# ansonb/RECON

Hardware: AMD Instinct MI355X
Metric: edges aggregated/sec (GAT fwd+bwd) on synthetic KG-context graphs (higher is better)
Workload: dtype f32

## Files before the change

include/recon_hip.h:

```cpp
#ifndef RECON_HIP_H
#define RECON_HIP_H

#include <stddef.h>
#include <stdint.h>

#ifdef __cplusplus
extern "C" {
#endif

#define RECON_ABI_VERSION 2

enum {
    RECON_OK = 0,
    RECON_ERR_INVALID = -1,
    RECON_ERR_UNSUPPORTED = -2,
    RECON_ERR_LAUNCH = -3,
    RECON_ERR_WORKSPACE = -4
};

typedef void* recon_stream_t;

int recon_version(void);
const char* recon_error_string(int code);

// ... 108 lines not shown
typedef struct {
    int32_t N, E;
    int32_t F, R, D, H;
    int32_t concat;
    float alpha;
    const float* x;
    const float* edge_embed;
    const float* a;
    const float* a_2;
    const float* keep;
    float* u;
    float* c_node;
    float* c_rel;
    float* V;
    float* sigma;
    float* Z;
    float* Zk;
    float* out;
    int32_t ld_out;
    void* a_split;
    int32_t split_mode;
    float keep_max;
    void* aux;
    const int32_t* ee_index;
    int32_t ee_rows;
    int32_t io_bf16;
} recon_gat_atp_args;
int recon_gat_atp_bf16_io_supported(int32_t F, int32_t R, int32_t D, int32_t H);

size_t recon_gat_atp_split_bytes(int32_t F, int32_t R, int32_t D, int32_t H);
int recon_gat_atp_f16x2_supported(int32_t F, int32_t R, int32_t D, int32_t H);
int recon_gat_atp_supported(int32_t N, int32_t E, int32_t F, int32_t R, int32_t D, int32_t H);
int32_t recon_gat_atp_instance(int32_t F, int32_t R, int32_t H);
int recon_gat_atp_fwd(const recon_graph* g, const recon_gat_atp_args* args, recon_stream_t stream);
int recon_gat_atp_scores(const recon_graph* g, const recon_gat_atp_args* args, recon_stream_t stream);
int recon_gat_atp_aggregate(const recon_graph* g, const recon_gat_atp_args* args, recon_stream_t stream);
int recon_gat_atp_project(const recon_graph* g, const recon_gat_atp_args* args, recon_stream_t stream);

typedef struct {
    recon_gat_atp_args fwd;
    const float* grad_out;
    int32_t ld_gout;
    float* g_h;
    float* g_V;
    float* g_sigma;
    float* Gxs;
    float* gxd;
    float* Gs;
    float* g_u;
    float* q;
    float* partial;
    float* partial2;
    float* g_x;
    float* g_edge_embed;
    float* g_a;
    float* g_a_2;
    void* gh_split;
    int32_t g_ee_bf16;
} recon_gat_atp_bwd_args;
int recon_gat_atp_bwd_gee_bf16_supported(int32_t F, int32_t R, int32_t D, int32_t H);

size_t recon_gat_atp_bwd_split_bytes(int32_t N, int32_t D, int32_t H);

size_t recon_gat_atp_bwd_partial_floats(int32_t N, int32_t E, int32_t F, int32_t R, int32_t D, int32_t H);
size_t recon_gat_atp_bwd_partial2_floats(int32_t N, int32_t E, int32_t F, int32_t R, int32_t D, int32_t H);
int recon_gat_atp_bwd_ride_plan(int32_t NR, int32_t N, int32_t E, int32_t F, int32_t R, int32_t D, int32_t H, int32_t* plan );
// ... 449 lines not shown
```

recon_amd/_lib.py:

```python
import ctypes as C
import os

_HERE = os.path.dirname(os.path.abspath(__file__))
LIB_PATH = os.environ.get("RECON_HIP_LIB") or os.path.join(_HERE, "csrc", "librecon_hip.so")

ERRORS = {0: "ok", -1: "invalid argument", -2: "unsupported shape", -3: "kernel launch failed",
          -4: "workspace too small"}

c_f32p = C.c_void_p
c_i32p = C.c_void_p
c_i64p = C.c_void_p


class ReconGraph(C.Structure):
    _fields_ = [("N", C.c_int32), ("E", C.c_int32),
                ("rowptr_dst", c_i32p), ("eid", c_i32p), ("src", c_i32p), ("dst", c_i32p),
                ("rowptr_src", c_i32p), ("slot_by_src", c_i32p),
                ("hub_chunk", C.c_int32), ("n_hub", C.c_int32), ("n_piece", C.c_int32),
                ("hub_node", c_i32p), ("hub_ptr", c_i32p), ("piece", c_i32p),
                ("n_hub_src", C.c_int32), ("n_piece_src", C.c_int32), ("hub_node_src", c_i32p), ("hub_ptr_src", c_i32p), ("piece_src", c_i32p),
                ("hub_ws", c_f32p), ("hub_ws_floats", C.c_int64),
                ("n_rows", C.c_int32), ("row_node", c_i32p), ("rowptr_rows", c_i32p), ("node_row", c_i32p)]


# ... 108 lines not shown
    ("recon_error_string", C.c_char_p, [C.c_int]),
    ("recon_graph_workspace_bytes", C.c_size_t, [C.c_int32, C.c_int32]),
    ("recon_graph_build", C.c_int, [c_i64p, c_i64p, C.POINTER(ReconGraph), C.c_void_p, C.c_size_t, C.c_void_p]),
    ("recon_graph_hubs_count", C.c_int, [C.POINTER(ReconGraph), C.c_int32, C.c_void_p, C.POINTER(C.c_int32), C.c_void_p]),
    ("recon_graph_build_checked", C.c_int, [c_i64p, c_i64p, C.POINTER(ReconGraph), C.c_void_p, C.c_size_t, C.c_void_p, C.c_void_p]),
    ("recon_graph_hubs_count_checked", C.c_int, [C.POINTER(ReconGraph), C.c_int32, C.c_void_p, C.POINTER(C.c_int32), C.c_void_p, C.POINTER(C.c_int32), C.c_void_p]),
    ("recon_graph_build_counted", C.c_int, [c_i64p, c_i64p, C.POINTER(ReconGraph), C.c_void_p, C.c_size_t, C.c_void_p, C.c_int32, C.c_void_p]),
    ("recon_graph_hubs_read", C.c_int, [C.POINTER(ReconGraph), C.c_void_p, C.POINTER(C.c_int32), C.c_void_p, C.POINTER(C.c_int32), C.c_void_p]),
    ("recon_graph_hubs_fill", C.c_int, [C.POINTER(ReconGraph), C.c_void_p]),
    ("recon_graph_counts_read", C.c_int, [C.POINTER(ReconGraph), C.c_void_p, C.POINTER(C.c_int32), C.POINTER(C.c_int32), C.c_void_p, C.POINTER(C.c_int32), C.c_void_p]),
    ("recon_graph_rows_compact", C.c_int, [C.POINTER(ReconGraph), C.c_void_p]),
    ("recon_edges_prune_batch", C.c_int, [C.c_void_p, C.c_int32, C.c_void_p, C.c_void_p, C.c_int64, C.c_void_p, C.c_int64, C.c_int32, C.c_void_p, C.c_void_p,
                                          C.c_void_p, C.c_void_p, C.c_void_p, C.c_void_p, C.c_void_p, C.c_void_p, C.c_int64, C.c_void_p]),
    ("recon_gat_atp_bwd_gee_bf16_supported", C.c_int, [C.c_int32, C.c_int32, C.c_int32, C.c_int32]),
    ("recon_slot_index", C.c_int, [C.c_void_p, C.c_void_p, C.c_int32, C.c_void_p, C.c_void_p, C.c_void_p]),
    ("recon_edges_prune", C.c_int, [C.c_void_p, C.c_void_p, C.c_int64, C.c_void_p, C.c_void_p, C.c_int64, C.c_void_p, C.c_int32, C.c_void_p, C.c_void_p,
                                    C.c_void_p, C.c_void_p, C.c_void_p, C.c_void_p, C.c_void_p, C.c_void_p]),
    ("recon_rows_expand", C.c_int, [C.c_void_p, C.c_int32, C.c_void_p, C.c_int32, C.c_int32, C.c_void_p, C.c_int32, C.c_void_p]),
    ("recon_graph_hub_ws_floats", C.c_size_t, [C.POINTER(ReconGraph), C.c_int32, C.c_int32, C.c_int32]),
    ("recon_spmm_rowsum_workspace_floats", C.c_size_t, [C.c_int32, C.c_int32]),
    ("recon_spmm_rowsum_fwd", C.c_int, [C.POINTER(ReconGraph), c_f32p, C.c_int32, c_f32p, c_f32p, C.c_void_p]),
    ("recon_spmm_rowsum_mod_fwd", C.c_int, [C.POINTER(ReconGraph), c_f32p, C.c_int32, C.c_int32, c_f32p, c_f32p, C.c_void_p]),
    ("recon_gather_rows_pair_fwd", C.c_int, [c_f32p, c_i64p, C.c_int64, C.c_int32, c_f32p, C.c_void_p]),
    ("recon_spmm_rowsum_bwd", C.c_int, [c_i64p, C.c_int64, c_f32p, C.c_int32, c_f32p, C.c_void_p]),
    ("recon_gat_fwd", C.c_int, [C.POINTER(ReconGraph), C.POINTER(GatFwdArgs), C.c_void_p]),
    ("recon_gat_project", C.c_int, [C.POINTER(ReconGraph), C.POINTER(GatFwdArgs), C.c_void_p]),
    ("recon_gat_edge_fwd", C.c_int, [C.POINTER(ReconGraph), C.POINTER(GatFwdArgs), C.c_void_p]),
    ("recon_gat_edge_instance", C.c_int32, [C.c_int32] * 2),
    ("recon_gat_bwd_partial_floats", C.c_size_t, [C.c_int32] * 6),
    ("recon_gat_bwd", C.c_int, [C.POINTER(ReconGraph), C.POINTER(GatBwdArgs), C.c_void_p]),
    ("recon_gat_atp_supported", C.c_int, [C.c_int32] * 6),
    ("recon_gat_atp_f16x2_supported", C.c_int, [C.c_int32] * 4),
    ("recon_gat_atp_instance", C.c_int32, [C.c_int32] * 3),
    ("recon_gat_atp_fwd", C.c_int, [C.POINTER(ReconGraph), C.POINTER(GatAtpArgs), C.c_void_p]),
    ("recon_gat_atp_scores", C.c_int, [C.POINTER(ReconGraph), C.POINTER(GatAtpArgs), C.c_void_p]),
    ("recon_gat_atp_aggregate", C.c_int, [C.POINTER(ReconGraph), C.POINTER(GatAtpArgs), C.c_void_p]),
    ("recon_gat_atp_project", C.c_int, [C.POINTER(ReconGraph), C.POINTER(GatAtpArgs), C.c_void_p]),
    ("recon_gat_atp_bwd_partial_floats", C.c_size_t, [C.c_int32] * 6),
    ("recon_gat_atp_bwd_partial2_floats", C.c_size_t, [C.c_int32] * 6),
    ("recon_gat_atp_bwd_ride_plan", C.c_int, [C.c_int32] * 7 + [C.POINTER(C.c_int32)]),
    ("recon_gat_atp_bwd", C.c_int, [C.POINTER(ReconGraph), C.POINTER(GatAtpBwdArgs), C.c_void_p]),
    ("recon_gat_atp_bwd_phase", C.c_int, [C.POINTER(ReconGraph), C.POINTER(GatAtpBwdArgs), C.c_int32, C.c_void_p]),
    ("recon_block_adjacency_fwd", C.c_int, [c_f32p, c_f32p, C.c_int32, C.c_int32, C.c_int32, c_f32p, C.c_void_p]),
    ("recon_block_adjacency_bwd_workspace_floats", C.c_size_t, [C.c_int32] * 3),
    ("recon_block_adjacency_bwd", C.c_int, [c_f32p, C.c_int32, C.c_int32, C.c_int32, c_f32p, c_f32p, c_f32p, C.c_void_p]),
    ("recon_propagate_fwd", C.c_int, [C.POINTER(PropArgs), C.c_void_p]),
    ("recon_propagate_bwd", C.c_int, [C.POINTER(PropBwdArgs), C.c_void_p]),
    ("recon_propagate_form", C.c_int, [C.POINTER(PropArgs)]),
    ("recon_propagate_instance", C.c_int32, [C.POINTER(PropArgs)]),
    ("recon_propagate_bwd_instance", C.c_int32, [C.POINTER(PropBwdArgs)]),
    ("recon_propagate_b16_instance", C.c_int32, [C.POINTER(PropB16Args), C.c_int32]),
    ("recon_propagate_identity_ws_floats", C.c_size_t, [C.c_int32]),
    ("recon_propagate_ws_bytes", C.c_size_t, [C.POINTER(PropArgs)]),
    ("recon_propagate_bwd_ws_floats", C.c_size_t, [C.POINTER(PropArgs)]),
    ("recon_propagate_bwd_chain_ws_floats", C.c_size_t, [C.POINTER(PropArgs)]),
    ("recon_propagate_b16_form", C.c_int, [C.POINTER(PropB16Args)]),
    ("recon_propagate_b16_fwd", C.c_int, [C.POINTER(PropB16Args), C.c_void_p]),
    ("recon_propagate_b16_bwd", C.c_int, [C.POINTER(PropB16BwdArgs), C.c_void_p]),
    ("recon_propagate_b16_bwd_diag_elems", C.c_size_t, [C.POINTER(PropB16Args)]),
    ("recon_block_adjacency_b16_fwd", C.c_int, [C.c_void_p, C.c_void_p, C.c_int32, C.c_int32, C.c_int32, C.c_void_p, C.c_void_p]),
    ("recon_block_adjacency_b16_bwd_workspace_floats", C.c_size_t, [C.c_int32]),
    ("recon_block_adjacency_b16_bwd", C.c_int, [C.c_void_p, C.c_int32, C.c_int32, C.c_int32, C.c_void_p, C.c_void_p, c_f32p, C.c_void_p]),
    ("recon_rel_rows_mm", C.c_int, [C.c_void_p] * 4 + [C.c_int32] * 4 + [C.c_void_p] * 2),
    ("recon_rel_rows_mm_wgrad", C.c_int, [C.c_void_p] * 4 + [C.c_int32] * 3 + [C.c_void_p] * 2),
    ("recon_rel_translation_supported", C.c_int, [C.c_int64, C.c_int32, C.c_int32, C.c_int32]),
    ("recon_rel_translation_saved_bytes", C.c_size_t, [C.c_int64, C.c_int32, C.c_int32]),
# ... 305 lines not shown
```

recon_amd/csrc/config.hip:

```cpp
#include <mutex>
#include <stdlib.h>
#include <string.h>
#include "recon_common.h"

namespace recon {
namespace {
const char* const kNames[CFG_COUNT] = {
    "RECON_GCN_FUSED", "RECON_GCN_FUSED_BWD", "RECON_GEMM_CFG", "RECON_GEMM_LIN", "RECON_GEMM_SPLITK", "RECON_GEMM_XCD", "RECON_PROP_B16",
    "RECON_PROP_B16_YPOST", "RECON_PROP_BWD", "RECON_PROP_BWD_CHAIN", "RECON_PROP_BWD_WIDE", "RECON_PROP_FWD", "RECON_PROP_LDS_KB", "RECON_ATP_ROW_SCALE",
    "RECON_GRAPH_SMALL", "RECON_KG_NHOP", "RECON_HX2_RING", "RECON_K2_LDS_RING", "RECON_K2_PERSIST"};
char g_val[CFG_COUNT][32];
bool g_set[CFG_COUNT];
std::once_flag g_once;

void store(int k, const char* v) {
    g_set[k] = v != nullptr;
    if (v) { strncpy(g_val[k], v, sizeof(g_val[k]) - 1); g_val[k][sizeof(g_val[k]) - 1] = '\0'; }
}
void load_env() {
    for (int k = 0; k < CFG_COUNT; ++k) store(k, getenv(kNames[k]));
}
int key_of(const char* name) {
    if (!name) return -1;
    for (int k = 0; k < CFG_COUNT; ++k) if (strcmp(name, kNames[k]) == 0) return k;
    return -1;
}
}

const char* cfg(CfgKey k) {
    std::call_once(g_once, load_env);
    return g_set[k] ? g_val[k] : nullptr;
}
int cfg_int(CfgKey k, int dflt) { const char* v = cfg(k); return v ? atoi(v) : dflt; }
char cfg_char(CfgKey k) { const char* v = cfg(k); return v ? v[0] : '\0'; }
}

namespace recon {
namespace {
int32_t* g_nan[16] = {};
bool g_nan_any = false;
}
int32_t* nan_flag() {
    if (!g_nan_any) return nullptr;
// ... 27 lines not shown
```

recon_amd/csrc/gat_atp.hip:

```cpp
#include <math.h>
#include <stdlib.h>
#include "recon_common.h"

#include <type_traits>

namespace recon {
namespace {

constexpr int kBlock = 256;

__device__ __forceinline__ int xcd_block(int b, int nb) {
    const int q = nb >> 3, r = nb & 7, x = b & 7, i = b >> 3;
    return (x < r ? x * (q + 1) : r * (q + 1) + (x - r) * q) + i;
}
template <int VEC, bool B16>
__device__ __forceinline__ void load_in(float (&r)[VEC], const float* base, int64_t e) {
    if constexpr (!B16) {
        load_vec<VEC>(r, base + e);
    } else {
        const uint16_t* b = reinterpret_cast<const uint16_t*>(base) + e;
        if constexpr (VEC == 4) {
            const uint2 t = *reinterpret_cast<const uint2*>(b);
            r[0] = __builtin_bit_cast(float, t.x << 16); r[1] = __builtin_bit_cast(float, t.x & 0xffff0000u);
            r[2] = __builtin_bit_cast(float, t.y << 16); r[3] = __builtin_bit_cast(float, t.y & 0xffff0000u);
// ... 84 lines not shown
    }
    red[threadIdx.x] = s;
    __syncthreads();
    for (int off = 128; off > 0; off >>= 1) {
        if (threadIdx.x < off) red[threadIdx.x] += red[threadIdx.x + off];
        __syncthreads();
    }
    if (threadIdx.x == 0 && ga2) ga2[h * D + d] = red[0];
}

__global__ void __launch_bounds__(256) k_atp_weights_finish(const float* __restrict__ partial, int32_t splits, int32_t W, int32_t D, int32_t H,
                                                            const float* __restrict__ a, const float* __restrict__ a2,
                                                            const float* __restrict__ gu, float* __restrict__ ga, float* __restrict__ ga2,
                                                            uint32_t* __restrict__ rezero, int32_t rezero_words) {
    __shared__ float tile[32][33];
    if (rezero && blockIdx.x == 0)
        for (int i = threadIdx.x; i < rezero_words; i += 256) rezero[i] = 0u;
    const int tw = (W + 31) / 32, td = (D + 31) / 32, ntile = tw * td * H;
    if (static_cast<int>(blockIdx.x) < ntile) {
        const int c8 = blockIdx.x & 7, b = c8 * (ntile >> 3) + min(c8, ntile & 7) + (blockIdx.x >> 3);
        const int h = b / (td * tw), m0 = ((b / td) % tw) * 32, n0 = (b % td) * 32;
        const int tx = threadIdx.x & 31, ty = threadIdx.x >> 5;
        const int64_t MN = static_cast<int64_t>(W) * D;
        const float* pz = partial + static_cast<int64_t>(h) * splits * MN;
        float acc[4] = {0.f, 0.f, 0.f, 0.f};
        int64_t off[4];
        bool ok[4];
#pragma unroll
        for (int i = 0; i < 4; ++i) {
            const int m = m0 + ty + 8 * i, n = n0 + tx;
            ok[i] = m < W && n < D;
            off[i] = ok[i] ? static_cast<int64_t>(m) * D + n : 0;
        }
        for (int z = 0; z < splits; ++z) {
#pragma unroll
            for (int i = 0; i < 4; ++i) acc[i] += pz[z * MN + off[i]];
        }
#pragma unroll
        for (int i = 0; i < 4; ++i) tile[ty + 8 * i][tx] = ok[i] ? acc[i] : 0.f;
        __syncthreads();
#pragma unroll
        for (int i = 0; i < 4; ++i) {
            const int n = n0 + ty + 8 * i, m = m0 + tx;
            if (m < W && n < D)
                ga[(static_cast<int64_t>(h) * D + n) * W + m] = fmaf(a2[h * D + n], gu[static_cast<int64_t>(h) * W + m], tile[tx][ty + 8 * i]);
        }
    } else if (ga2) {
        const int lane = threadIdx.x & 63, wave = threadIdx.x >> 6;
        const int r0 = (static_cast<int>(blockIdx.x) - ntile) * 8 + wave * 2;
#pragma unroll
        for (int i = 0; i < 2; ++i) {
            const int r = r0 + i;
            if (r >= H * D) break;
            const int h = r / D;
            float sum = 0.f;
            for (int w = 4 * lane; w < W; w += 256) {
                const float4 av = *reinterpret_cast<const float4*>(a + static_cast<int64_t>(r) * W + w);
                const float4 gv = *reinterpret_cast<const float4*>(gu + static_cast<int64_t>(h) * W + w);
                sum = fmaf(av.x, gv.x, fmaf(av.y, gv.y, fmaf(av.z, gv.z, fmaf(av.w, gv.w, sum))));
            }
#pragma unroll
            for (int off = 32; off > 0; off >>= 1) sum += __shfl_xor(sum, off, 64);
            if (lane == 0) ga2[r] = sum;
        }
    }
}

__global__ void __launch_bounds__(256) k_elu_grad_q(const float* __restrict__ gy, int32_t ld_gy, const float* __restrict__ y,
                                                    int32_t ld_y, int32_t N, int32_t H, int32_t D, int32_t concat,
// ... 1209 lines not shown
        p.Gs_dst[static_cast<int64_t>(node) * 2 * H + lane] += tot;
    }
    for (int c = lane * VEC; c < F; c += 64 * VEC) {
        float o[VEC];
        load_vec<VEC>(o, p.gxd + static_cast<int64_t>(node) * F + c);
        for (int h = 0; h < H; ++h) {
            const float sh = lane_bcast(tot, h);
            float ud[VEC];
            load_vec<VEC>(ud, p.u + static_cast<int64_t>(h) * W + c);
#pragma unroll
            for (int v = 0; v < VEC; ++v) o[v] = fmaf(sh, ud[v], o[v]);
        }
        store_vec<VEC>(p.gxd + static_cast<int64_t>(node) * F + c, o);
    }
}

struct AtpSrcK {
    const int32_t* rowptr_src; const int32_t* slot_by_src; const float* Gxs; const float* gxd; const float* gsigma;
    float* g_x; float* Gs_src;
    const float* u; int32_t W;
    int32_t N, F, H;
    int32_t hub_chunk, n_piece;
    const int4* piece;
    float* hubP;
    const int32_t* node_row;
};
template <int VEC, int KR>
__device__ __forceinline__ void atp_src_wave(const AtpSrcK& p, int bx, int nbx) {
    const int lane = threadIdx.x & 63;
    const int wave = __builtin_amdgcn_readfirstlane(threadIdx.x >> 6);
    const int npb = (p.n_piece + kBlock / 64 - 1) / (kBlock / 64);
    const int widx = bx * (kBlock / 64) + wave;
    const bool is_piece = bx < npb;
    int node = xcd_block(bx - npb, nbx - npb) * (kBlock / 64) + wave;
    int beg, end;
    if (is_piece) {
        if (widx >= p.n_piece) return;
        const int4 pc = p.piece[widx]; node = pc.x; beg = pc.y; end = pc.z;
    } else {
        if (node >= p.N) return;
        beg = p.rowptr_src[node]; end = p.rowptr_src[node + 1];
        if (p.hub_chunk && end - beg > p.hub_chunk) return;
    }
    const int F = p.F, H = p.H;
    const int drow = (p.node_row && !is_piece) ? p.node_row[node] : node;
    float acc[KR][VEC];
#pragma unroll
    for (int r = 0; r < KR; ++r) {
#pragma unroll
        for (int v = 0; v < VEC; ++v) acc[r][v] = 0.f;
        const int c = (r * 64 + lane) * VEC;
        if (!is_piece && c < F && p.g_x && drow >= 0) load_vec<VEC>(acc[r], p.gxd + static_cast<int64_t>(drow) * F + c);
    }
    float gs = 0.f;
    constexpr int U = 4;
    const int hl = lane < H ? lane : 0;
    for (int c0 = beg; c0 < end; c0 += 64) {
        const int cn = min(64, end - c0);
        const int slotv = p.slot_by_src[c0 + min(lane, cn - 1)];
        for (int j0 = 0; j0 < cn; j0 += U) {
            int slot[U];
#pragma unroll
            for (int u = 0; u < U; ++u) slot[u] = __builtin_amdgcn_readlane(slotv, min(j0 + u, cn - 1));
            float g4[U], t[U][KR][VEC];
#pragma unroll
            for (int u = 0; u < U; ++u) {
                g4[u] = p.gsigma[static_cast<int64_t>(slot[u]) * H + hl];
                if (p.g_x) {
#pragma unroll
                    for (int r = 0; r < KR; ++r) {
                        const int c = (r * 64 + lane) * VEC;
                        load_vec<VEC>(t[u][r], p.Gxs + static_cast<int64_t>(slot[u]) * F + (c < F ? c : 0));
                    }
                }
            }
#pragma unroll
            for (int u = 0; u < U; ++u) {
                if (j0 + u < cn) {
                    gs += g4[u];
                    if (p.g_x) {
#pragma unroll
                        for (int r = 0; r < KR; ++r)
#pragma unroll
                            for (int v = 0; v < VEC; ++v) acc[r][v] += t[u][r][v];
                    }
                }
            }
        }
    }
    float* gs_out = is_piece ? p.hubP + static_cast<int64_t>(widx) * (F + H) + F : p.Gs_src + static_cast<int64_t>(node) * 2 * H + H;
    float* row_out = is_piece ? p.hubP + static_cast<int64_t>(widx) * (F + H) : p.g_x + static_cast<int64_t>(node) * F;
    if (lane < H) gs_out[lane] = gs;
    if (!is_piece && p.g_x) {
        constexpr int HBK = KR <= 2 ? 8 : 2;
        for (int hb = 0; hb < H; hb += HBK) {
            float us[HBK][KR][VEC];
#pragma unroll
            for (int t = 0; t < HBK; ++t) {
                const float* uh = p.u + static_cast<int64_t>(min(hb + t, H - 1)) * p.W + F;
#pragma unroll
                for (int r = 0; r < KR; ++r) {
                    const int c = (r * 64 + lane) * VEC;
                    load_vec<VEC>(us[t][r], uh + (c < F ? c : 0));
                }
            }
#pragma unroll
            for (int t = 0; t < HBK; ++t) {
                const float sh = hb + t < H ? lane_bcast(gs, min(hb + t, 63)) : 0.f;
#pragma unroll
                for (int r = 0; r < KR; ++r)
#pragma unroll
                    for (int v = 0; v < VEC; ++v) acc[r][v] = fmaf(sh, us[t][r][v], acc[r][v]);
            }
        }
    }
    if (p.g_x) {
#pragma unroll
        for (int r = 0; r < KR; ++r) {
            const int c = (r * 64 + lane) * VEC;
            if (c < F) {
                if (is_piece && ((F + H) % VEC)) {
#pragma unroll
                    for (int v = 0; v < VEC; ++v) row_out[c + v] = acc[r][v];
                } else store_vec<VEC>(row_out + c, acc[r]);
            }
        }
    }
}

template <int VEC, int KR>
__global__ void __launch_bounds__(kBlock) k_gat_atp_src(const AtpSrcK p) { atp_src_wave<VEC, KR>(p, blockIdx.x, gridDim.x); }

__global__ void __launch_bounds__(kBlock) k_gat_atp_hub_src(const AtpSrcK p, const int32_t* __restrict__ hub_node, const int32_t* __restrict__ hub_ptr,
                                                            int32_t n_hub) {
    const int lane = threadIdx.x & 63;
    const int F = p.F, H = p.H;
    const int stripes = (F + 63) / 64;
    const int idx = blockIdx.x * (kBlock / 64) + __builtin_amdgcn_readfirstlane(threadIdx.x >> 6);
    if (idx >= n_hub * stripes) return;
    const int t = idx / stripes, c = (idx - t * stripes) * 64 + lane;
    const int node = hub_node[t], p0 = hub_ptr[t], p1 = hub_ptr[t + 1];
    float gsl[1] = {0.f};
    if (lane < H) sum_pieces<1>(gsl, p.hubP + F + lane, F + H, p0, p1);
    if (c < H) p.Gs_src[static_cast<int64_t>(node) * 2 * H + H + c] = gsl[0];
    if (!p.g_x) return;
    const int drow = p.node_row ? p.node_row[node] : node;
    float a[1] = {(c < F && drow >= 0) ? p.gxd[static_cast<int64_t>(drow) * F + c] : 0.f};
    if (c < F) sum_pieces<1>(a, p.hubP + c, F + H, p0, p1);
    for (int h = 0; h < H; ++h) a[0] = fmaf(lane_bcast(gsl[0], h), p.u[static_cast<int64_t>(h) * p.W + F + (c < F ? c : 0)], a[0]);
    if (c < F) p.g_x[static_cast<int64_t>(node) * F + c] = a[0];
}


struct SkinnyJob { const float* G; const float* X; const int32_t* gather; float* partial; int32_t ldg, nj, rows, K, rpb, nb; };
struct SkinnySrc { const int32_t* rowptr_src; const int32_t* slot_by_src; const float* gsigma; };
template <int NJ, bool B16, bool SRC>
__device__ __forceinline__ void skinny_block(const SkinnyJob& jb, int bid, float (&red)[NJ][256], float* __restrict__ gsl, const SkinnySrc& sr, bool src) {
    constexpr int RPI = 4;
    const float* __restrict__ G = jb.G;
// ... 135 lines not shown

#define ATP_DISPATCH(S, CALL)                                                                              \
    do {                                                                                                   \
        const int key_ = atp_key(S);                                                                       \
        switch (key_) {                                                                                    \
            case 4010: CALL(4, 1, 1); break; case 4011: CALL(4, 1, 2); break; case 4012: CALL(4, 1, 4); break; case 4013: CALL(4, 1, 8); break; \
            case 4020: CALL(4, 2, 1); break; case 4021: CALL(4, 2, 2); break; case 4022: CALL(4, 2, 4); break;   \
            case 4040: CALL(4, 4, 1); break; case 4041: CALL(4, 4, 2); break; case 4080: CALL(4, 8, 1); break;   \
            case 2010: CALL(2, 1, 1); break; case 2011: CALL(2, 1, 2); break; case 2012: CALL(2, 1, 4); break; case 2013: CALL(2, 1, 8); break; \
            case 2020: CALL(2, 2, 1); break; case 2021: CALL(2, 2, 2); break; case 2022: CALL(2, 2, 4); break; case 2023: CALL(2, 2, 8); break; \
            case 2040: CALL(2, 4, 1); break; case 2041: CALL(2, 4, 2); break; case 2042: CALL(2, 4, 4); break;   \
            case 2080: CALL(2, 8, 1); break; case 2081: CALL(2, 8, 2); break;                                   \
            default: return RECON_ERR_UNSUPPORTED;                                                         \
        }                                                                                                  \
    } while (0)

int check_atp(const recon_graph* g, const recon_gat_atp_args* a) {
    if (!g || !a) return RECON_ERR_INVALID;
    if (a->N != g->N || a->E != g->E) return RECON_ERR_INVALID;
    if (a->N < 0 || a->E < 0 || a->F <= 0 || a->R <= 0 || a->D <= 0 || a->H <= 0) return RECON_ERR_INVALID;
    if (a->ld_out < a->H * a->D) return RECON_ERR_INVALID;
    if (!a->x || !a->a || !a->a_2 || !a->u || !a->c_node || !a->V || !a->out) return RECON_ERR_INVALID;
    if (a->E > 0 && (!a->edge_embed || !a->c_rel)) return RECON_ERR_INVALID;
    if (a->H > 4096) return RECON_ERR_UNSUPPORTED;
    if (a->ee_index && a->E > 0 && a->ee_rows <= 0) return RECON_ERR_INVALID;
    return RECON_OK;
}

}
}

using namespace recon;

static int64_t k2_resident_blocks(int kr, int ht, size_t lds_bytes) {
    static int cus = 0;
    if (cus == 0) {
        int dev = 0, n = 0;
        if (hipGetDevice(&dev) != hipSuccess || hipDeviceGetAttribute(&n, hipDeviceAttributeMultiprocessorCount, dev) != hipSuccess || n <= 0) n = 256;
        cus = n;
    }
    const int waves_per_simd = (kr * ht >= 8 && kr >= 8) ? 1 : ((kr >= 4 || (kr * ht >= 8 && kr >= 2)) ? 2 : 3);
    int per_cu = waves_per_simd;
    const int by_lds = static_cast<int>((160 * 1024) / (lds_bytes + 256));
    if (by_lds < per_cu) per_cu = by_lds < 1 ? 1 : by_lds;
    return static_cast<int64_t>(cus) * per_cu / 8 * 8;
}

extern "C" int recon_gat_atp_supported(int32_t N, int32_t E, int32_t F, int32_t R, int32_t D, int32_t H) {
    (void)N; (void)E; (void)D;
    AtpShape s;
    if (F <= 0 || R <= 0 || H <= 0 || H > 32) return 0;
    if (!atp_shape(F, R, H, &s)) return 0;
    if (2 * H > 64) return 0;
    const int64_t W = 2LL * F + R, mx = F > R ? F : R;
    if (4 * H * W > 64 * 1024 || 8LL * H * (mx + 4) > 64 * 1024) return 0;
    return 1;
}

extern "C" int32_t recon_gat_atp_instance(int32_t F, int32_t R, int32_t H) {
    AtpShape s;
    if (F <= 0 || R <= 0 || H <= 0 || !atp_shape(F, R, H, &s)) return -1;
    return atp_key(s);
}

static size_t split_part_bytes(int64_t rows, int32_t K, int32_t H) { return align_up(static_cast<size_t>(3) * H * rows * bx3_kp(K) * 2, 256); }
extern "C" size_t recon_gat_atp_split_bytes(int32_t F, int32_t R, int32_t D, int32_t H) {
    if (F <= 0 || R <= 0 || D <= 0 || H <= 0) return 256;
    const int32_t W = 2 * F + R;
    return split_part_bytes(D, W, H) + split_part_bytes(W, D, H);
}

static bool atp_hx2_shape(int32_t F, int32_t R, int32_t D, int32_t H) {
    const int64_t W = 2LL * F + R;
// ... 373 lines not shown
                                  else if (LRC && lring) hipLaunchKernelGGL((k_gat_atp_bwd<V_, K_, H_, false, LRC>), grid, dim3(kBlock), lds_run, st, p);              \
                                  else hipLaunchKernelGGL((k_gat_atp_bwd<V_, K_, H_>), grid, dim3(kBlock), lds_run, st, p); } while (0)
        p.persist = (p.n_piece == 0 && cfg_char(CFG_K2_PERSIST) != '0') ? 1 : 0;
        if (p.persist) {
            const int64_t need = ceil_div64(NR, kBlock / 64);
            int64_t nb = k2_resident_blocks(s.kr, s.ht, lds_run);
            if (nb > need) nb = (need + 7) / 8 * 8;
            grid = dim3(static_cast<unsigned>(nb));
        } else {
            grid = dim3(static_cast<unsigned>(ceil_div64(NR, kBlock / 64) + ceil_div64(p.n_piece, kBlock / 64)));
        }
        ATP_DISPATCH(s, CALL_BWD);
#undef CALL_BWD
        if (hubs) {
            const dim3 gh(static_cast<unsigned>(ceil_div64(g->n_hub, kBlock / 64)));
            if (s.vec == 4) hipLaunchKernelGGL((k_gat_atp_hub_bwd<4>), gh, dim3(kBlock), 0, st, p, g->hub_node, g->hub_ptr, g->n_hub);
            else hipLaunchKernelGGL((k_gat_atp_hub_bwd<2>), gh, dim3(kBlock), 0, st, p, g->hub_node, g->hub_ptr, g->n_hub);
        }
        RECON_CHECK_LAUNCH();
    }
    {
        AtpSrcK p;
        p.rowptr_src = g->rowptr_src; p.slot_by_src = g->slot_by_src; p.Gxs = b->Gxs; p.gxd = b->gxd; p.gsigma = b->g_sigma;
        p.g_x = b->g_x; p.Gs_src = b->Gs; p.u = a->u; p.W = W;
        p.N = N; p.F = F; p.H = H; p.node_row = rw.node_row;
        const bool hubs = g->hub_chunk > 0 && g->n_hub_src > 0 && g->n_piece_src > 0 && g->hub_node_src && g->hub_ptr_src && g->piece_src && g->hub_ws;
        if (hubs && static_cast<size_t>(g->hub_ws_floats) < recon_graph_hub_ws_floats(g, F, R, H)) return RECON_ERR_WORKSPACE;
        p.hub_chunk = hubs ? g->hub_chunk : 0; p.n_piece = hubs ? g->n_piece_src : 0;
        p.piece = reinterpret_cast<const int4*>(g->piece_src); p.hubP = g->hub_ws;
        const bool want_u = b->g_a || b->g_a_2;
        if (want_u && !b->g_a) return RECON_ERR_INVALID;
        const size_t lds_src = static_cast<size_t>(skinny_rpb(N)) * H * sizeof(float);
        const bool share = want_u && H <= 8 && !hubs && lds_src <= kSkinnySrcLdsMax && (!a->io_bf16 || s.vec == 4);
        const int nsrc = static_cast<int>(ceil_div64(N, kBlock / 64) + ceil_div64(p.n_piece, kBlock / 64));
        const bool ride = share && hx2 && row_inv && (phases & RECON_ATP_BWD_WEIGHTS) && !(phases & RECON_ATP_BWD_EARLY_SUM);
        SkinnyJob sj[3];
        int nb_total = 0;
        auto launch_src = [&]() -> int {
            const dim3 grid(static_cast<unsigned>(nsrc + (share ? nb_total : 0)));
            const SkinnySrc sr{g->rowptr_src, g->slot_by_src, b->g_sigma};
#define CALL_SRC(V_, K_) do { if (!share) hipLaunchKernelGGL((k_gat_atp_src<V_, K_>), grid, dim3(kBlock), 0, st, p);                                          \
                              else if (V_ == 4 && a->io_bf16) hipLaunchKernelGGL((k_gat_atp_src_skinny<4, K_, true>), grid, dim3(kBlock), lds_src, st, p, nsrc, sj[0], sj[1], sj[2], sr); \
                              else hipLaunchKernelGGL((k_gat_atp_src_skinny<V_, K_, false>), grid, dim3(kBlock), lds_src, st, p, nsrc, sj[0], sj[1], sj[2], sr); } while (0)
            switch (s.vec * 10 + s.kr) {
                case 41: CALL_SRC(4, 1); break; case 42: CALL_SRC(4, 2); break; case 44: CALL_SRC(4, 4); break; case 48: CALL_SRC(4, 8); break;
                case 21: CALL_SRC(2, 1); break; case 22: CALL_SRC(2, 2); break; case 24: CALL_SRC(2, 4); break; default: CALL_SRC(2, 8); break;
            }
#undef CALL_SRC
            if (hubs) hipLaunchKernelGGL(k_gat_atp_hub_src, dim3(static_cast<unsigned>(ceil_div64(1LL * g->n_hub_src * ceil_div64(F, 64), kBlock / 64))), dim3(kBlock), 0, st, p,
                                         g->hub_node_src, g->hub_ptr_src, g->n_hub_src);
            return RECON_OK;
        };
        if (!share) launch_src();
        if (want_u) {
            struct Prod { const float* G; int ldg, nj; const float* X; const int32_t* gather; int rows, K, P; int64_t S1, S2; float* out; };
            const int32_t* ee_gather = a->ee_index ? a->ee_index : g->eid;
            const size_t third = recon_gat_atp_bwd_partial2_floats(N, E, F, R, D, H) / 3;
            auto run_jobs = [&](const Prod* pr, int count) {
                SkinnyRedJob rj[3];
                int nj_max = 0, nr_total = 0;
                nb_total = 0;
                for (int i = 0; i < 3; ++i) {
                    sj[i] = SkinnyJob{nullptr, nullptr, nullptr, nullptr, 0, 0, 0, 0, 1, 0};
                    rj[i] = SkinnyRedJob{nullptr, nullptr, 0, 0, 0, 0, 0, 1, 0};
                    if (i >= count) continue;
                    const Prod& q = pr[i];
                    if (q.rows <= 0) {
                        for (int j = 0; j < q.nj; ++j) (void)hipMemsetAsync(q.out + (j % q.P) * q.S1 + (j / q.P) * q.S2, 0, sizeof(float) * q.K, st);
                        continue;
                    }
                    const int rpb = skinny_rpb(q.rows);
                    const int nb = static_cast<int>(ceil_div64(q.rows, rpb));
                    float* part = b->partial2 + i * third;
                    sj[i] = SkinnyJob{q.G, q.X, q.gather, part, q.ldg, q.nj, q.rows, q.K, rpb, nb};
                    rj[i] = SkinnyRedJob{part, q.out, q.S1, q.S2, nb, q.nj, q.K, q.P, skinny_red_blocks(q.nj, q.K)};
                    if (q.nj > nj_max) nj_max = q.nj;
// ... 76 lines not shown
```

recon_amd/csrc/recon_common.h:

```cpp
#pragma once
#include <hip/hip_runtime.h>
#include <stdint.h>
#include "recon_hip.h"

#define RECON_CHECK_LAUNCH()                                   \
    do {                                                       \
        if (hipGetLastError() != hipSuccess) return RECON_ERR_LAUNCH; \
    } while (0)

static inline hipStream_t as_stream(recon_stream_t s) { return reinterpret_cast<hipStream_t>(s); }
static inline int64_t ceil_div64(int64_t a, int64_t b) { return (a + b - 1) / b; }
static inline size_t align_up(size_t x, size_t a) { return (x + a - 1) / a * a; }

namespace recon {

constexpr int kWave = 64;

enum CfgKey { CFG_GCN_FUSED, CFG_GCN_FUSED_BWD, CFG_GEMM_CFG, CFG_GEMM_LIN, CFG_GEMM_SPLITK, CFG_GEMM_XCD, CFG_PROP_B16, CFG_PROP_B16_YPOST,
              CFG_PROP_BWD, CFG_PROP_BWD_CHAIN, CFG_PROP_BWD_WIDE, CFG_PROP_FWD, CFG_PROP_LDS_KB, CFG_ATP_ROW_SCALE, CFG_GRAPH_SMALL, CFG_KG_NHOP,
              CFG_HX2_RING, CFG_K2_LDS_RING, CFG_K2_PERSIST, CFG_COUNT };
const char* cfg(CfgKey k);
int cfg_int(CfgKey k, int dflt);
char cfg_char(CfgKey k);
int32_t* nan_flag();

template <int CTRL>
__device__ __forceinline__ float dpp_mov(float v) {
    return __builtin_bit_cast(float, __builtin_amdgcn_update_dpp(0, __builtin_bit_cast(int, v), CTRL, 0xf, 0xf, true));
}

__device__ __forceinline__ float swap_add32(float a, float b) {
    const auto r = __builtin_amdgcn_permlane32_swap(__builtin_bit_cast(unsigned, a), __builtin_bit_cast(unsigned, b), false, false);
    const unsigned r0 = r[0], r1 = r[1];
    return __builtin_bit_cast(float, r0) + __builtin_bit_cast(float, r1);
}
__device__ __forceinline__ float swap_add16(float a, float b) {
    const auto r = __builtin_amdgcn_permlane16_swap(__builtin_bit_cast(unsigned, a), __builtin_bit_cast(unsigned, b), false, false);
    const unsigned r0 = r[0], r1 = r[1];
    return __builtin_bit_cast(float, r0) + __builtin_bit_cast(float, r1);
}
template <int G>
__device__ __forceinline__ float group_sum(float v) {
    static_assert(G == 4 || G == 8 || G == 16 || G == 32 || G == 64, "group width");
    v += dpp_mov<0xB1>(v);
    v += dpp_mov<0x4E>(v);
    if constexpr (G >= 8) v += dpp_mov<0x141>(v);
    if constexpr (G >= 16) v += dpp_mov<0x140>(v);
    if constexpr (G >= 32) v = swap_add16(v, v);
    if constexpr (G >= 64) v = swap_add32(v, v);
    return v;
}

template <int NV>
// ... 320 lines not shown
```

Before: 84.49 million.

## Make GAT ATP source-gradient kernel persistent with XCD-chunked nodes and prefetch

When there are no hub pieces, the source-side backward kernel now launches only as many blocks as can be resident, sized from an occupancy query and rounded to multiples of eight. Each wave then loops over nodes within a per-XCD contiguous chunk, and it prefetches the next node's row bounds and first slot indices while the current node is still being processed. The split-reduction loop is also unrolled four deep so several partial loads are in flight at once. This aims to cut block launch and tail overhead and hide index-load latency, at the cost of possible load imbalance across the fixed chunks and extra register pressure.

```diff
diff --git a/include/recon_hip.h b/include/recon_hip.h
--- a/include/recon_hip.h
+++ b/include/recon_hip.h
@@ -164,6 +164,7 @@
 int recon_gat_atp_f16x2_supported(int32_t F, int32_t R, int32_t D, int32_t H);
 int recon_gat_atp_supported(int32_t N, int32_t E, int32_t F, int32_t R, int32_t D, int32_t H);
 int32_t recon_gat_atp_instance(int32_t F, int32_t R, int32_t H);
+int32_t recon_atp_resident_blocks(int32_t per_cu, int32_t shared, int32_t need);
 int recon_gat_atp_fwd(const recon_graph* g, const recon_gat_atp_args* args, recon_stream_t stream);
 int recon_gat_atp_scores(const recon_graph* g, const recon_gat_atp_args* args, recon_stream_t stream);
 int recon_gat_atp_aggregate(const recon_graph* g, const recon_gat_atp_args* args, recon_stream_t stream);
diff --git a/recon_amd/_lib.py b/recon_amd/_lib.py
--- a/recon_amd/_lib.py
+++ b/recon_amd/_lib.py
@@ -164,6 +164,7 @@
     ("recon_gat_atp_supported", C.c_int, [C.c_int32] * 6),
     ("recon_gat_atp_f16x2_supported", C.c_int, [C.c_int32] * 4),
     ("recon_gat_atp_instance", C.c_int32, [C.c_int32] * 3),
+    ("recon_atp_resident_blocks", C.c_int32, [C.c_int32] * 3),
     ("recon_gat_atp_fwd", C.c_int, [C.POINTER(ReconGraph), C.POINTER(GatAtpArgs), C.c_void_p]),
     ("recon_gat_atp_scores", C.c_int, [C.POINTER(ReconGraph), C.POINTER(GatAtpArgs), C.c_void_p]),
     ("recon_gat_atp_aggregate", C.c_int, [C.POINTER(ReconGraph), C.POINTER(GatAtpArgs), C.c_void_p]),
diff --git a/recon_amd/csrc/config.hip b/recon_amd/csrc/config.hip
--- a/recon_amd/csrc/config.hip
+++ b/recon_amd/csrc/config.hip
@@ -8,7 +8,7 @@
 const char* const kNames[CFG_COUNT] = {
     "RECON_GCN_FUSED", "RECON_GCN_FUSED_BWD", "RECON_GEMM_CFG", "RECON_GEMM_LIN", "RECON_GEMM_SPLITK", "RECON_GEMM_XCD", "RECON_PROP_B16",
     "RECON_PROP_B16_YPOST", "RECON_PROP_BWD", "RECON_PROP_BWD_CHAIN", "RECON_PROP_BWD_WIDE", "RECON_PROP_FWD", "RECON_PROP_LDS_KB", "RECON_ATP_ROW_SCALE",
-    "RECON_GRAPH_SMALL", "RECON_KG_NHOP", "RECON_HX2_RING", "RECON_K2_LDS_RING", "RECON_K2_PERSIST"};
+    "RECON_GRAPH_SMALL", "RECON_KG_NHOP", "RECON_HX2_RING", "RECON_K2_LDS_RING", "RECON_K2_PERSIST", "RECON_ATP_RESIDENT_CAP"};
 char g_val[CFG_COUNT][32];
 bool g_set[CFG_COUNT];
 std::once_flag g_once;
diff --git a/recon_amd/csrc/gat_atp.hip b/recon_amd/csrc/gat_atp.hip
--- a/recon_amd/csrc/gat_atp.hip
+++ b/recon_amd/csrc/gat_atp.hip
@@ -140,9 +140,22 @@
             ok[i] = m < W && n < D;
             off[i] = ok[i] ? static_cast<int64_t>(m) * D + n : 0;
         }
-        for (int z = 0; z < splits; ++z) {
-#pragma unroll
-            for (int i = 0; i < 4; ++i) acc[i] += pz[z * MN + off[i]];
+        constexpr int ZU = 4;
+        for (int z0 = 0; z0 < splits; z0 += ZU) {
+            float v[ZU][4];
+#pragma unroll
+            for (int k = 0; k < ZU; ++k) {
+                const int64_t zo = static_cast<int64_t>(min(z0 + k, splits - 1)) * MN;
+#pragma unroll
+                for (int i = 0; i < 4; ++i) v[k][i] = pz[zo + off[i]];
+            }
+#pragma unroll
+            for (int k = 0; k < ZU; ++k) {
+                if (z0 + k < splits) {
+#pragma unroll
+                    for (int i = 0; i < 4; ++i) acc[i] += v[k][i];
+                }
+            }
         }
 #pragma unroll
         for (int i = 0; i < 4; ++i) tile[ty + 8 * i][tx] = ok[i] ? acc[i] : 0.f;
@@ -1418,17 +1431,29 @@
     const int npb = (p.n_piece + kBlock / 64 - 1) / (kBlock / 64);
     const int widx = bx * (kBlock / 64) + wave;
     const bool is_piece = bx < npb;
-    int node = xcd_block(bx - npb, nbx - npb) * (kBlock / 64) + wave;
+    const bool persist = p.n_piece == 0;
+    const int xcd = bx & 7, nchunk = (p.N + 7) >> 3;
+    const int node_hi = persist ? min(p.N, (xcd + 1) * nchunk) : p.N, node_stride = ((nbx + 7 - xcd) >> 3) * (kBlock / 64);
+    int node = persist ? xcd * nchunk + (bx >> 3) * (kBlock / 64) + wave : xcd_block(bx - npb, nbx - npb) * (kBlock / 64) + wave;
     int beg, end;
     if (is_piece) {
         if (widx >= p.n_piece) return;
         const int4 pc = p.piece[widx]; node = pc.x; beg = pc.y; end = pc.z;
     } else {
-        if (node >= p.N) return;
+        if (node >= node_hi) return;
         beg = p.rowptr_src[node]; end = p.rowptr_src[node + 1];
         if (p.hub_chunk && end - beg > p.hub_chunk) return;
     }
     const int F = p.F, H = p.H;
+    auto first_slots = [&](int b, int e) { return b < e ? p.slot_by_src[b + min(lane, min(64, e - b) - 1)] : 0; };
+    int slotv0 = first_slots(beg, end);
+#pragma unroll 1
+    for (;;) {
+    node = __builtin_amdgcn_readfirstlane(node); beg = __builtin_amdgcn_readfirstlane(beg); end = __builtin_amdgcn_readfirstlane(end);
+    const int nnode = persist ? node + node_stride : p.N;
+    const bool more = nnode < node_hi;
+    int nbeg = 0, nend = 0, nslotv = 0;
+    if (more) { nbeg = p.rowptr_src[nnode]; nend = p.rowptr_src[nnode + 1]; }
     const int drow = (p.node_row && !is_piece) ? p.node_row[node] : node;
     float acc[KR][VEC];
 #pragma unroll
@@ -1441,39 +1466,46 @@
     float gs = 0.f;
     constexpr int U = 4;
     const int hl = lane < H ? lane : 0;
-    for (int c0 = beg; c0 < end; c0 += 64) {
-        const int cn = min(64, end - c0);
-        const int slotv = p.slot_by_src[c0 + min(lane, cn - 1)];
-        for (int j0 = 0; j0 < cn; j0 += U) {
-            int slot[U];
-#pragma unroll
-            for (int u = 0; u < U; ++u) slot[u] = __builtin_amdgcn_readlane(slotv, min(j0 + u, cn - 1));
-            float g4[U], t[U][KR][VEC];
-#pragma unroll
-            for (int u = 0; u < U; ++u) {
-                g4[u] = p.gsigma[static_cast<int64_t>(slot[u]) * H + hl];
+    auto edges = [&](int slotv, int cn, int j0, auto first) {
+        int slot[U];
+#pragma unroll
+        for (int u = 0; u < U; ++u) slot[u] = __builtin_amdgcn_readlane(slotv, min(j0 + u, cn - 1));
+        float g4[U], t[U][KR][VEC];
+#pragma unroll
+        for (int u = 0; u < U; ++u) {
+            g4[u] = p.gsigma[static_cast<int64_t>(slot[u]) * H + hl];
+            if (p.g_x) {
+#pragma unroll
+                for (int r = 0; r < KR; ++r) {
+                    const int c = (r * 64 + lane) * VEC;
+                    load_vec<VEC>(t[u][r], p.Gxs + static_cast<int64_t>(slot[u]) * F + (c < F ? c : 0));
+                }
+            }
+        }
+        if constexpr (decltype(first)::value) nslotv = first_slots(nbeg, nend);
+#pragma unroll
+        for (int u = 0; u < U; ++u) {
+            if (j0 + u < cn) {
+                gs += g4[u];
                 if (p.g_x) {
 #pragma unroll
-                    for (int r = 0; r < KR; ++r) {
-                        const int c = (r * 64 + lane) * VEC;
-                        load_vec<VEC>(t[u][r], p.Gxs + static_cast<int64_t>(slot[u]) * F + (c < F ? c : 0));
-                    }
-                }
-            }
-#pragma unroll
-            for (int u = 0; u < U; ++u) {
-                if (j0 + u < cn) {
-                    gs += g4[u];
-                    if (p.g_x) {
-#pragma unroll
-                        for (int r = 0; r < KR; ++r)
-#pragma unroll
-                            for (int v = 0; v < VEC; ++v) acc[r][v] += t[u][r][v];
-                    }
-                }
-            }
-        }
-    }
+                    for (int r = 0; r < KR; ++r)
+#pragma unroll
+                        for (int v = 0; v < VEC; ++v) acc[r][v] += t[u][r][v];
+                }
+            }
+        }
+    };
+    if (beg < end) {
+        const int cn0 = min(64, end - beg);
+        edges(slotv0, cn0, 0, std::true_type{});
+        for (int j0 = U; j0 < cn0; j0 += U) edges(slotv0, cn0, j0, std::false_type{});
+        for (int c0 = beg + 64; c0 < end; c0 += 64) {
+            const int cn = min(64, end - c0);
+            const int slotv = p.slot_by_src[c0 + min(lane, cn - 1)];
+            for (int j0 = 0; j0 < cn; j0 += U) edges(slotv, cn, j0, std::false_type{});
+        }
+    } else nslotv = first_slots(nbeg, nend);
     float* gs_out = is_piece ? p.hubP + static_cast<int64_t>(widx) * (F + H) + F : p.Gs_src + static_cast<int64_t>(node) * 2 * H + H;
     float* row_out = is_piece ? p.hubP + static_cast<int64_t>(widx) * (F + H) : p.g_x + static_cast<int64_t>(node) * F;
     if (lane < H) gs_out[lane] = gs;
@@ -1511,6 +1543,9 @@
                 } else store_vec<VEC>(row_out + c, acc[r]);
             }
         }
+    }
+    if (!more) break;
+    node = nnode; beg = nbeg; end = nend; slotv0 = nslotv;
     }
 }
 
@@ -1712,13 +1747,38 @@
 
 using namespace recon;
 
-static int64_t k2_resident_blocks(int kr, int ht, size_t lds_bytes) {
+static int device_cus() {
     static int cus = 0;
     if (cus == 0) {
         int dev = 0, n = 0;
         if (hipGetDevice(&dev) != hipSuccess || hipDeviceGetAttribute(&n, hipDeviceAttributeMultiprocessorCount, dev) != hipSuccess || n <= 0) n = 256;
         cus = n;
     }
+    return cus;
+}
+
+extern "C" int32_t recon_atp_resident_blocks(int32_t per_cu, int32_t shared, int32_t need) {
+    if (need <= 0) return 0;
+    if (per_cu < 1) per_cu = 1;
+    int64_t nb = static_cast<int64_t>(device_cus()) * per_cu / (shared ? 2 : 1) / 8 * 8;
+    if (nb < 8) nb = 8;
+    const int cap = cfg_int(CFG_ATP_RESIDENT_CAP, 0);
+    if (cap > 0 && nb > cap) nb = cap >= 8 ? cap / 8 * 8 : 8;
+    return nb < need ? static_cast<int32_t>(nb) : need;
+}
+struct OccMemo { size_t lds = ~static_cast<size_t>(0); int per_cu = 0; };
+template <typename Kern>
+static int kernel_blocks_per_cu(OccMemo& memo, Kern kern, int block, size_t lds) {
+    if (memo.lds != lds || memo.per_cu == 0) {
+        int n = 0;
+        if (hipOccupancyMaxActiveBlocksPerMultiprocessor(&n, kern, block, lds) != hipSuccess || n < 1) n = 1;
+        memo.per_cu = n; memo.lds = lds;
+    }
+    return memo.per_cu;
+}
+
+static int64_t k2_resident_blocks(int kr, int ht, size_t lds_bytes) {
+    const int cus = device_cus();
     const int waves_per_simd = (kr * ht >= 8 && kr >= 8) ? 1 : ((kr >= 4 || (kr * ht >= 8 && kr >= 2)) ? 2 : 3);
     int per_cu = waves_per_simd;
     const int by_lds = static_cast<int>((160 * 1024) / (lds_bytes + 256));
@@ -2158,16 +2218,22 @@
         if (want_u && !b->g_a) return RECON_ERR_INVALID;
         const size_t lds_src = static_cast<size_t>(skinny_rpb(N)) * H * sizeof(float);
         const bool share = want_u && H <= 8 && !hubs && lds_src <= kSkinnySrcLdsMax && (!a->io_bf16 || s.vec == 4);
-        const int nsrc = static_cast<int>(ceil_div64(N, kBlock / 64) + ceil_div64(p.n_piece, kBlock / 64));
+        int nsrc = static_cast<int>(ceil_div64(N, kBlock / 64) + ceil_div64(p.n_piece, kBlock / 64));
         const bool ride = share && hx2 && row_inv && (phases & RECON_ATP_BWD_WEIGHTS) && !(phases & RECON_ATP_BWD_EARLY_SUM);
         SkinnyJob sj[3];
         int nb_total = 0;
         auto launch_src = [&]() -> int {
-            const dim3 grid(static_cast<unsigned>(nsrc + (share ? nb_total : 0)));
             const SkinnySrc sr{g->rowptr_src, g->slot_by_src, b->g_sigma};
-#define CALL_SRC(V_, K_) do { if (!share) hipLaunchKernelGGL((k_gat_atp_src<V_, K_>), grid, dim3(kBlock), 0, st, p);                                          \
-                              else if (V_ == 4 && a->io_bf16) hipLaunchKernelGGL((k_gat_atp_src_skinny<4, K_, true>), grid, dim3(kBlock), lds_src, st, p, nsrc, sj[0], sj[1], sj[2], sr); \
-                              else hipLaunchKernelGGL((k_gat_atp_src_skinny<V_, K_, false>), grid, dim3(kBlock), lds_src, st, p, nsrc, sj[0], sj[1], sj[2], sr); } while (0)
+            dim3 grid;
+#define SRC_GRID(KERN_, LDS_) do { if (p.n_piece == 0) { static OccMemo occ;                                                                                    \
+                                                         const int32_t need8 = static_cast<int32_t>(ceil_div64(N, 8 * (kBlock / 64)) * 8);                                            \
+                                                         nsrc = ((recon_atp_resident_blocks(kernel_blocks_per_cu(occ, KERN_, kBlock, LDS_), share && nb_total > 0, need8) + 7) / 8 * 8); } \
+                                   grid = dim3(static_cast<unsigned>(nsrc + (share ? nb_total : 0))); } while (0)
+#define CALL_SRC(V_, K_) do { if (!share) { SRC_GRID((k_gat_atp_src<V_, K_>), 0); hipLaunchKernelGGL((k_gat_atp_src<V_, K_>), grid, dim3(kBlock), 0, st, p); } \
+                              else if (V_ == 4 && a->io_bf16) { SRC_GRID((k_gat_atp_src_skinny<4, K_, true>), lds_src);                                          \
+                                                                hipLaunchKernelGGL((k_gat_atp_src_skinny<4, K_, true>), grid, dim3(kBlock), lds_src, st, p, nsrc, sj[0], sj[1], sj[2], sr); } \
+                              else { SRC_GRID((k_gat_atp_src_skinny<V_, K_, false>), lds_src);                                                                   \
+                                     hipLaunchKernelGGL((k_gat_atp_src_skinny<V_, K_, false>), grid, dim3(kBlock), lds_src, st, p, nsrc, sj[0], sj[1], sj[2], sr); } } while (0)
             switch (s.vec * 10 + s.kr) {
                 case 41: CALL_SRC(4, 1); break; case 42: CALL_SRC(4, 2); break; case 44: CALL_SRC(4, 4); break; case 48: CALL_SRC(4, 8); break;
                 case 21: CALL_SRC(2, 1); break; case 22: CALL_SRC(2, 2); break; case 24: CALL_SRC(2, 4); break; default: CALL_SRC(2, 8); break;
diff --git a/recon_amd/csrc/recon_common.h b/recon_amd/csrc/recon_common.h
--- a/recon_amd/csrc/recon_common.h
+++ b/recon_amd/csrc/recon_common.h
@@ -18,7 +18,7 @@
 
 enum CfgKey { CFG_GCN_FUSED, CFG_GCN_FUSED_BWD, CFG_GEMM_CFG, CFG_GEMM_LIN, CFG_GEMM_SPLITK, CFG_GEMM_XCD, CFG_PROP_B16, CFG_PROP_B16_YPOST,
               CFG_PROP_BWD, CFG_PROP_BWD_CHAIN, CFG_PROP_BWD_WIDE, CFG_PROP_FWD, CFG_PROP_LDS_KB, CFG_ATP_ROW_SCALE, CFG_GRAPH_SMALL, CFG_KG_NHOP,
-              CFG_HX2_RING, CFG_K2_LDS_RING, CFG_K2_PERSIST, CFG_COUNT };
+              CFG_HX2_RING, CFG_K2_LDS_RING, CFG_K2_PERSIST, CFG_ATP_RESIDENT_CAP, CFG_COUNT };
 const char* cfg(CfgKey k);
 int cfg_int(CfgKey k, int dflt);
 char cfg_char(CfgKey k);
```

Result: slower. 82.82 million (-2.0%).
